# Unalome81/IEEE-802.11-OFDM-QPSK-Simulator

Hardware: NVIDIA B200
Metric: OFDM symbols/s, TX+AWGN+RX chain (BER/EVM sweep) (higher is better)
Workload: dtype f32+f64

## Files before the change

### ieee-802.11-ofdm-qpsk-simulator_b200/csrc/ofdm_sweep.cuh

```cuda
#pragma once
#include "ofdm_chain.cuh"

namespace ofdm {

struct SweepParams {
    const float2 *in;
    const float *g;
    const float *power;
    const uint32_t *tx_bits;
    long n_frames;
    int n_snr;
    float radius_scale;
    float evm_guard;
    float snr_lin[kMaxSnr];
    ofdm_counters *counters;
    unsigned long long *replayed;
};

struct alignas(16) SweepWarp {
    float2 tile[kWarpTile];
    float2 fx[4][kWin];
    float2 fn[4][kWin];
    StreamStage<true> st[kStages];
    uint64_t bar[kStages];
    float norm[8];
};
static_assert(sizeof(SweepWarp) % 16 == 0 && offsetof(SweepWarp, st) % 16 == 0 && offsetof(SweepWarp, norm) % 16 == 0, "SweepWarp alignment");

__device__ __forceinline__ float modulus_up(float2 z)
{
    float r;
    asm("sqrt.approx.ftz.f32 %0, %1;" : "=f"(r) : "f"(fmaf(z.x, z.x, z.y * z.y)));
    return fmaf(r, 1.000004f, 2e-19f);
}

__constant__ unsigned char c_sweep_pair[32] = { 1,  2,  5,  8, 11, 16, 19, 41, 44, 45, 46, 52, 54, 55, 58, 63,
                                                3,  4, 10, 12, 17, 18, 22, 23, 25, 47, 48, 53, 56, 59, 61, 62};
__constant__ unsigned char c_sweep_single[16] = { 6, 14, 15, 20, 26, 40, 49, 50,    9, 13, 24, 38, 39, 42, 51, 60};

struct SweepItems {
    int bin[2];
    int f_off[3];
    float k4[3];
    int word[3];
    int shift[3];
};

__device__ __forceinline__ SweepItems make_sweep_items(int lane)
{
    SweepItems c;
    c.bin[0] = c_sweep_pair[lane];
    c.bin[1] = c_sweep_single[(lane >> 4) * 8 + (lane & 7)];
#pragma unroll
    for (int t = 0; t < 3; ++t) {
        const int bin = c.bin[t >> 1], sym = t == 2 ? (lane >> 3) & 1 : t;
        const int d = c_tab.bin_data[bin];
        c.f_off[t] = sym * kWin + bin;
        c.k4[t] = 4.f * (0.5f * (float)c_tab.bin_lts[bin]);
        c.word[t] = sym * 3 + (d >> 4);
        c.shift[t] = 2 * (d & 15);
    }
    return c;
}

constexpr int kSweepWarps = 6;

template <int ARITH>
__global__ void __launch_bounds__(kSweepWarps * 32, 2) k_sweep_lin(SweepParams p)
{
    constexpr int LEVEL = ARITH == kArithChecked ? 2 : 1;
    constexpr int kWarps = kSweepWarps;
    extern __shared__ __align__(128) unsigned char s_raw[];
    const int lane = threadIdx.x & 31, warp = threadIdx.x >> 5, grp = lane >> 3, u = lane & 7;
    const int warp_u = __shfl_sync(0xffffffffu, warp, 0);
    SweepWarp &ws = reinterpret_cast<SweepWarp *>(s_raw)[warp];
    SweepWarp &ws_u = reinterpret_cast<SweepWarp *>(s_raw)[warp_u];
    float2 *tile = ws.tile + grp * kGroupPitch;
    Tw<false> tw; tw.load(u);
    const SweepItems ic = make_sweep_items(lane);
    constexpr int len = 320;
    const long stride = (long)gridDim.x * kWarps;
    const long f_first = (long)blockIdx.x * kWarps + warp_u;
    const double q = (double)kQpsk;
    const double ref2_frame = 96.0 * (2.0 * q * q);
    const float inv_ref2 = (float)(1.0 / ref2_frame);
    constexpr uint32_t kBytes = 4 * 512 + 4 * 256;
    constexpr int kStep = 3;

    const uint32_t stage0 = tma::saddr(&ws_u.st[0]);
    const uint32_t bar0 = tma::saddr(&ws_u.bar[0]);
    auto issue = [&](long f, int s) {
        if (tma::elect_one()) {
            const uint32_t bar = bar0 + 8u * (uint32_t)s;
            const uint32_t dst = stage0 + (uint32_t)s * (uint32_t)sizeof(StreamStage<true>);
            const char *x = reinterpret_cast<const char *>(p.in) + f * (len * 8);
            const char *g = reinterpret_cast<const char *>(p.g) + f * (len * 4);
            const uint32_t gd = dst + 4 * kWin * 8;
            tma::expect_tx_addr(bar, kBytes);
            tma::bulk_addr(dst + 0 * kWin * 8, x + 32 * 8, 512, bar);
            tma::bulk_addr(dst + 1 * kWin * 8, x + 96 * 8, 512, bar);
            tma::bulk_addr(dst + 2 * kWin * 8, x + 176 * 8, 512, bar);
            tma::bulk_addr(dst + 3 * kWin * 8, x + 256 * 8, 512, bar);
            tma::bulk_addr(gd + 0 * kWin * 4, g + 32 * 4, 256, bar);
            tma::bulk_addr(gd + 1 * kWin * 4, g + 96 * 4, 256, bar);
            tma::bulk_addr(gd + 2 * kWin * 4, g + 176 * 4, 256, bar);
            tma::bulk_addr(gd + 3 * kWin * 4, g + 256 * 4, 256, bar);
        }
    };
    if (lane == 0) {
        for (int s = 0; s < kStages; ++s) tma::mbar_init(&ws.bar[s], 1);
        tma::fence_mbar_init();
    }
    __syncwarp();
    for (int s = 0; s < kStages; ++s)
        if (f_first + s * stride < p.n_frames) issue(f_first + s * stride, s);

    uint32_t m_i[2] = {0, 0}, m_q[2] = {0, 0}, m_b[2] = {0, 0}, m_ferr[2] = {0, 0};
    float m_e2[2] = {0.f, 0.f}, m_evm[2] = {0.f, 0.f};
    double d_e2[2] = {0.0, 0.0}, d_evm[2] = {0.0, 0.0};
    uint32_t n_done = 0;
    uint32_t k = 0;
    for (long f = f_first; f < p.n_frames; f += stride, ++k) {
        const int s = (int)(k & 1u);
        const uint32_t phase = (k >> 1) & 1u;
        const float P = p.power[f];
        const uint32_t *wb = p.tx_bits + f * 6;
        uint32_t txw[3];
#pragma unroll
        for (int t = 0; t < 3; ++t) txw[t] = wb[ic.word[t]];

        tma::wait_addr(bar0 + 8u * (uint32_t)s, phase);
        float2 v[8];
        float gz[8];
        float2 n2x = make_float2(0.f, 0.f);
        float n2g = 0.f;
#pragma unroll
        for (int i = 0; i < 8; ++i) {
            v[i] = ws.st[s].x[grp][u + 8 * i];
            gz[i] = ws.st[s].g[grp][u + 8 * i];
            n2x = __ffma2_rn(v[i], v[i], n2x);
            n2g = fmaf(gz[i], gz[i], n2g);
        }
        __syncwarp();
        if (f + kStages * stride < p.n_frames) issue(f + kStages * stride, s);
        fft64<false>(v, tw, tile, u);
#pragma unroll
        for (int j = 0; j < 8; ++j) ws.fx[grp][u + 8 * j] = v[j];
#pragma unroll
        for (int i = 0; i < 8; ++i) v[i] = make_float2(gz[i], 0.f);
        fft64<false>(v, tw, tile, u);
#pragma unroll
        for (int j = 0; j < 8; ++j) ws.fn[grp][u + 8 * j] = v[j];
        float2 nn = make_float2(n2x.x + n2x.y, n2g);
#pragma unroll
        for (int o = 1; o < 8; o <<= 1)
            nn = __fadd2_rn(nn, make_float2(__shfl_xor_sync(0xffffffffu, nn.x, o), __shfl_xor_sync(0xffffffffu, nn.y, o)));
        {
            float rx, rn;
            asm("sqrt.approx.ftz.f32 %0, %1;" : "=f"(rx) : "f"(nn.x));
            asm("sqrt.approx.ftz.f32 %0, %1;" : "=f"(rn) : "f"(nn.y));
            const bool ok = nn.x >= 1e-30f && nn.x < 1e20f && nn.y < 1e20f;
            const float inf = __int_as_float(0x7f800000);
            if (u == 0) { ws.norm[grp] = ok ? p.radius_scale * rx : inf; ws.norm[4 + grp] = ok ? p.radius_scale * rn : inf; }
        }
        __syncwarp();
        const float4 rX = *reinterpret_cast<const float4 *>(ws.norm), rN = *reinterpret_cast<const float4 *>(ws.norm + 4);
        const float rHX = rX.x + rX.y, rHN = rN.x + rN.y;
        float2 FX[3], FN[3], GX[2], GN[2];
        float c0[3], c1[3], c2[3], hcX[2], hcN[2];
#pragma unroll
        for (int e = 0; e < 2; ++e) {
            const int bin = ic.bin[e];
            GX[e] = cadd(ws.fx[0][bin], ws.fx[1][bin]);
            GN[e] = cadd(ws.fn[0][bin], ws.fn[1][bin]);
            if (LEVEL >= 2) { hcX[e] = modulus_up(GX[e]); hcN[e] = modulus_up(GN[e]); }
        }
#pragma unroll
        for (int t = 0; t < 3; ++t) {
            FX[t] = (&ws.fx[2][0])[ic.f_off[t]];
            FN[t] = (&ws.fn[2][0])[ic.f_off[t]];
            const bool sym0 = ic.f_off[t] < kWin;
            const float rFX = sym0 ? rX.z : rX.w, rFN = sym0 ? rN.z : rN.w;
            if (LEVEL >= 2) {
                const float faX = modulus_up(FX[t]), faN = modulus_up(FN[t]);
                const float hX = hcX[t >> 1], hN = hcN[t >> 1];
                const float A0 = hX + rHX, A1 = hN + rHN;
                c0[t] = fmaf(rFX, A0, fmaf(rHX, faX, 1.2e-7f * (faX * hX)));
                c1[t] = fmaf(rFX, A1, fmaf(rFN, A0, fmaf(rHX, faN, fmaf(rHN, faX, 1.2e-7f * fmaf(faX, hN, faN * hX)))));
                c2[t] = fmaf(rFN, A1, fmaf(rHN, faN, 1.2e-7f * (faN * hN)));
            } else { c0[t] = c1[t] = c2[t] = 0.f; }
        }
        __syncwarp();
        uint32_t gq[3];
#pragma unroll
        for (int t = 0; t < 3; ++t) {
            const uint32_t tp = txw[t] >> ic.shift[t];
            const uint32_t kb = __float_as_uint(ic.k4[t]) & 0x80000000u;
            const uint32_t fq = (tp << 31) ^ kb, fi = ((tp ^ (tp >> 1)) << 31) ^ kb;
            gq[t] = (tp >> 1) << 31;
            FX[t] = make_float2(__uint_as_float(__float_as_uint(FX[t].x) ^ fi), __uint_as_float(__float_as_uint(FX[t].y) ^ fq));
            FN[t] = make_float2(__uint_as_float(__float_as_uint(FN[t].x) ^ fi), __uint_as_float(__float_as_uint(FN[t].y) ^ fq));
        }
#pragma unroll
        for (int e = 0; e < 2; ++e) {
            GX[e].y = __uint_as_float(__float_as_uint(GX[e].y) ^ gq[2 * e]);
            GN[e].y = __uint_as_float(__float_as_uint(GN[e].y) ^ gq[2 * e]);
        }
        const uint32_t g_rel = gq[0] ^ gq[1];
        float sig_lo = 0.f, sig_hi = 0.f;
        if (lane < p.n_snr) sig_lo = __fsqrt_rn(__fdiv_rn(P, p.snr_lin[lane]));
        if (p.n_snr > 32 && lane + 32 < p.n_snr) sig_hi = __fsqrt_rn(__fdiv_rn(P, p.snr_lin[lane + 32]));
        auto sig_pos = [](int i) { return (i / 3) * 4 + i % 3; };
        float *sigs = reinterpret_cast<float *>(&ws.fn[1][0]);
        sigs[sig_pos(lane)] = sig_lo; sigs[sig_pos(lane + 32)] = sig_hi;
        if (lane < 2) sigs[sig_pos(64 + lane)] = 0.f;
        __syncwarp();

        uint2 *res = reinterpret_cast<uint2 *>(&ws.fn[0][0]);
        const float g2_limit = p.radius_scale * 1.58e6f;
        struct PointState { float sg, rH2, den_min4; float2 e2v; uint32_t pk; bool doubt; float2 G; float den, inv; };
        auto point_begin = [&](float sg) {
            PointState q;
            q.sg = sg;
            q.rH2 = fmaf(sg, rHN, rHX);
            const float gd = p.evm_guard * q.rH2;
            q.den_min4 = gd * gd;
            q.e2v = make_float2(0.f, 0.f);
            q.pk = 0; q.doubt = !(q.rH2 < g2_limit);
            return q;
        };
        auto point_item = [&](PointState &q, int t) {
            const float2 sg2 = make_float2(q.sg, q.sg);
            if (t != 1) {
                q.G = __ffma2_rn(sg2, GN[t >> 1], GX[t >> 1]);
                q.den = fmaf(q.G.x, q.G.x, q.G.y * q.G.y);
                asm("rcp.approx.ftz.f32 %0, %1;" : "=f"(q.inv) : "f"(q.den));
            }
            const float2 G = t == 1 ? make_float2(q.G.x, __uint_as_float(__float_as_uint(q.G.y) ^ g_rel)) : q.G;
            const float2 F = __ffma2_rn(sg2, FN[t], FX[t]);
            const float thr = fmaf(fmaf(c2[t], q.sg, c1[t]), q.sg, c0[t]);
            q.pk += process_bin_spec_den<LEVEL, true>(F, G, q.den, q.inv, 2.f, 0u, thr, q.rH2, q.den_min4, q.e2v, q.doubt);
        };
        uint32_t pk_raw[kStep];
        float e2_pend[kStep], red[kStep], red_in[kStep];
#pragma unroll
        for (int j = 0; j < kStep; ++j) { pk_raw[j] = 0; e2_pend[j] = 0.f; }
        auto red_issue = [&](int o) {
#pragma unroll
            for (int j = 0; j < kStep; ++j) red_in[j] = __shfl_xor_sync(0xffffffffu, red[j], o);
        };
        auto red_take = [&]() {
#pragma unroll
            for (int j = 0; j < kStep; ++j) red[j] += red_in[j];
        };
        uint64_t doubt_mask = 0;
        for (int si = 0, sk = 0; si < p.n_snr; si += kStep, sk += 4) {
            uint32_t pk_sum[kStep];
#pragma unroll
            for (int j = 0; j < kStep; ++j) { pk_sum[j] = __reduce_add_sync(0xffffffffu, pk_raw[j]); red[j] = e2_pend[j]; }
            red_issue(16);
            PointState q[kStep];
            const float4 sp = *reinterpret_cast<const float4 *>(sigs + sk);
            q[0] = point_begin(sp.x); q[1] = point_begin(sp.y); q[2] = point_begin(sp.z);
#pragma unroll
            for (int t = 0; t < 3; ++t) {
#pragma unroll
                for (int j = 0; j < kStep; ++j) {
                    const int n = t * kStep + j;
                    point_item(q[j], t);
                    if (n < 4) { red_take(); red_issue(8 >> n); }
                    else if (n == 4) red_take();
                }
            }
            if (lane == 0 && si > 0) {
#pragma unroll
                for (int j = 0; j < kStep; ++j) res[si - kStep + j] = make_uint2(pk_sum[j], __float_as_uint(red[j]));
            }
            uint32_t bits = 0;
#pragma unroll
            for (int j = 0; j < kStep; ++j) {
                pk_raw[j] = q[j].pk;
                e2_pend[j] = q[j].e2v.x + q[j].e2v.y;
                bits |= (uint32_t)q[j].doubt << j;
            }
            doubt_mask |= (uint64_t)bits << si;
        }
        {
            const int last = (p.n_snr - 1) / kStep * kStep;
#pragma unroll
            for (int j = 0; j < kStep; ++j) {
                const uint32_t pk_sum = __reduce_add_sync(0xffffffffu, pk_raw[j]);
                float r = e2_pend[j];
#pragma unroll
                for (int o = 16; o > 0; o >>= 1) r += __shfl_xor_sync(0xffffffffu, r, o);
                if (lane == 0) res[last + j] = make_uint2(pk_sum, __float_as_uint(r));
            }
        }
        {
            if (p.n_snr < 64) doubt_mask &= (1ull << p.n_snr) - 1ull;
            uint64_t todo = __reduce_or_sync(0xffffffffu, (uint32_t)doubt_mask);
            if (p.n_snr > 32) todo |= (uint64_t)__reduce_or_sync(0xffffffffu, (uint32_t)(doubt_mask >> 32)) << 32;
            __syncwarp();
            while (todo != 0) {
                const int si = __ffsll((long long)todo) - 1;
                todo &= todo - 1;
                const float sg = sigs[sig_pos(si)];
                bool replay = true;
                if (LEVEL >= 2) {
                    const float4 qX = *reinterpret_cast<const float4 *>(ws.norm), qN = *reinterpret_cast<const float4 *>(ws.norm + 4);
                    const float2 sg2 = make_float2(sg, sg);
                    const float rH2 = fmaf(sg, rHN, rHX);
                    const float gd = p.evm_guard * rH2, den_min4 = gd * gd;
                    bool doubt2 = false;
                    float2 e2w = make_float2(0.f, 0.f);
                    float2 G;
#pragma unroll
                    for (int t = 0; t < 3; ++t) {
                        if (t != 1) G = __ffma2_rn(sg2, GN[t >> 1], GX[t >> 1]);
                        const float2 Gt = t == 1 ? make_float2(G.x, __uint_as_float(__float_as_uint(G.y) ^ g_rel)) : G;
                        const float2 F = __ffma2_rn(sg2, FN[t], FX[t]);
                        const bool sym0 = ic.f_off[t] < kWin;
                        const float rF = fmaf(sg, sym0 ? qN.z : qN.w, sym0 ? qX.z : qX.w);
                        const float fa = modulus_up(F), hc = modulus_up(Gt);
                        const float thr = fmaf(rF, hc + rH2, fmaf(rH2, fa, 1.2e-7f * (fa * hc)));
                        process_bin_spec<LEVEL, true>(F, Gt, 2.f, 0u, thr, rH2, den_min4, e2w, doubt2);
                    }
                    replay = __any_sync(0xffffffffu, doubt2);
                }
                if (replay) {
                    const double sigma_d = __dsqrt_rn((double)__fdiv_rn(P, p.snr_lin[si]));
                    const uint2 r = stream_frame_replay<kNoiseInject>(p.in + f * len, p.g + f * len, wb, sigma_d, 0u, 0u, 0ull,
                                                                      ws.tile, &ws.fx[0][0], p.replayed);
                    const uint32_t pk_sum = __reduce_add_sync(0xffffffffu, r.x);
                    float e2 = __uint_as_float(r.y);
#pragma unroll
                    for (int o = 16; o > 0; o >>= 1) e2 += __shfl_xor_sync(0xffffffffu, e2, o);
                    if (lane == 0) res[si] = make_uint2(pk_sum, __float_as_uint(e2));
                }
            }
        }
        __syncwarp();
#pragma unroll
        for (int h = 0; h < 2; ++h) {
            if (h == 1 && p.n_snr <= 32) break;
            const uint2 r = res[lane + 32 * h];
            const bool mine = lane + 32 * h < p.n_snr;
            const uint32_t pk = mine ? r.x : 0u;
            const float e2 = mine ? __uint_as_float(r.y) : 0.f;
            float evm;
            asm("sqrt.approx.ftz.f32 %0, %1;" : "=f"(evm) : "f"(e2 * inv_ref2));
            m_i[h] += pk & 0xFFu; m_q[h] += (pk >> 8) & 0xFFu; m_b[h] += pk >> 16; m_ferr[h] += pk != 0u;
            m_e2[h] += e2; m_evm[h] += evm;
        }
        n_done += 1;
        if ((n_done & 63u) == 0u) {
#pragma unroll
            for (int h = 0; h < 2; ++h) { d_e2[h] += (double)m_e2[h]; d_evm[h] += (double)m_evm[h]; m_e2[h] = 0.f; m_evm[h] = 0.f; }
        }
    }
    if (n_done == 0) return;
#pragma unroll
    for (int h = 0; h < 2; ++h) {
        const int si = lane + 32 * h;
        if (si >= p.n_snr) continue;
        ofdm_counters *o = p.counters + si;
        const unsigned long long ti = m_i[h], tq = m_q[h], tb = m_b[h];
        atomicAdd(reinterpret_cast<unsigned long long *>(&o->bit_errors), ti + 2ull * tq - 2ull * tb);
        atomicAdd(reinterpret_cast<unsigned long long *>(&o->rail_errors), ti + tq);
        atomicAdd(reinterpret_cast<unsigned long long *>(&o->frames_in_error), (unsigned long long)m_ferr[h]);
        atomicAdd(reinterpret_cast<unsigned long long *>(&o->frames), (unsigned long long)n_done);
        atomicAdd(reinterpret_cast<unsigned long long *>(&o->bits), 192ull * n_done);
        atomicAdd(&o->sum_err2, d_e2[h] + (double)m_e2[h]);
        atomicAdd(&o->sum_ref2, ref2_frame * (double)n_done);
        atomicAdd(&o->sum_evm_lin, d_evm[h] + (double)m_evm[h]);
    }
}

inline size_t sweep_smem_bytes(int warps) { return sizeof(SweepWarp) * warps; }

}
```

Measured before the change: 10.61 billion.

## Replace per-SNR shuffle reductions with shared-memory transpose and specialized item kernel

Replaces the interleaved butterfly shuffle reduction of EVM partials with per-lane writes of partials into a shared-memory matrix, then each lane sums its own SNR row with paired float adds. Adds a specialized inlined sweep_item that computes the decision, margin and error with packed float2 ops, and folds the doubt check into a three-way NaN-propagating min over margins. Enlarges the per-warp shared struct with dedicated sig and pk arrays, which raises shared memory use and may reduce occupancy. Replay results are now held in the owning lane's registers instead of a shared result array.

```diff
diff --git a/ieee-802.11-ofdm-qpsk-simulator_b200/csrc/ofdm_sweep.cuh b/ieee-802.11-ofdm-qpsk-simulator_b200/csrc/ofdm_sweep.cuh
--- a/ieee-802.11-ofdm-qpsk-simulator_b200/csrc/ofdm_sweep.cuh
+++ b/ieee-802.11-ofdm-qpsk-simulator_b200/csrc/ofdm_sweep.cuh
@@ -17,21 +17,50 @@
     unsigned long long *replayed;
 };
 
+constexpr int kSweepRows = kMaxSnr + 2;
+constexpr int kPartPitch = 36;
+constexpr int kSweepSlots = (kMaxSnr + 2) / 3 * 4;
+
 struct alignas(16) SweepWarp {
     float2 tile[kWarpTile];
     float2 fx[4][kWin];
     float2 fn[4][kWin];
+    float part_tail[kSweepRows * kPartPitch - 2 * (kWarpTile + 8 * kWin)];
+    float sig[kSweepSlots];
+    uint32_t pk[kSweepSlots];
     StreamStage<true> st[kStages];
     uint64_t bar[kStages];
     float norm[8];
 };
-static_assert(sizeof(SweepWarp) % 16 == 0 && offsetof(SweepWarp, st) % 16 == 0 && offsetof(SweepWarp, norm) % 16 == 0, "SweepWarp alignment");
+static_assert(sizeof(SweepWarp) % 16 == 0 && offsetof(SweepWarp, st) % 16 == 0 && offsetof(SweepWarp, norm) % 16 == 0 &&
+              offsetof(SweepWarp, sig) % 16 == 0 && offsetof(SweepWarp, pk) % 16 == 0, "SweepWarp alignment");
+static_assert(offsetof(SweepWarp, part_tail) == 2 * (kWarpTile + 8 * kWin) * sizeof(float) &&
+              offsetof(SweepWarp, sig) == kSweepRows * kPartPitch * sizeof(float), "the partials run from tile to sig");
 
 __device__ __forceinline__ float modulus_up(float2 z)
 {
     float r;
     asm("sqrt.approx.ftz.f32 %0, %1;" : "=f"(r) : "f"(fmaf(z.x, z.x, z.y * z.y)));
     return fmaf(r, 1.000004f, 2e-19f);
+}
+
+__device__ __forceinline__ uint32_t sweep_item(float2 F, float2 G, float inv, float thr, float &margin, float2 &e2)
+{
+    const float2 pt = __fmul2_rn(make_float2(G.y, G.y), make_float2(F.y, F.x));
+    const float2 S = __ffma2_rn(make_float2(G.x, G.x), F, make_float2(pt.x, -pt.y));
+    const uint32_t ei = __float_as_uint(S.x) >> 31, eq = __float_as_uint(S.y) >> 31;
+    margin = fminf(fabsf(S.x), fabsf(S.y)) - thr;
+    const float2 U = __fmul2_rn(S, make_float2(inv, inv));
+    const float2 D = __ffma2_rn(U, make_float2(2.f, 2.f), make_float2(__uint_as_float(0xBF3504F3u), __uint_as_float(0xBF3504F3u)));
+    e2 = __ffma2_rn(D, D, e2);
+    return ei | (eq << 8) | ((ei & eq) << 16);
+}
+
+__device__ __forceinline__ float min3_nan(float a, float b, float c)
+{
+    float r;
+    asm("min.NaN.f32 %0, %1, %2, %3;" : "=f"(r) : "f"(a), "f"(b), "f"(c));
+    return r;
 }
 
 __constant__ unsigned char c_sweep_pair[32] = { 1,  2,  5,  8, 11, 16, 19, 41, 44, 45, 46, 52, 54, 55, 58, 63,
@@ -211,14 +240,14 @@
         if (lane < p.n_snr) sig_lo = __fsqrt_rn(__fdiv_rn(P, p.snr_lin[lane]));
         if (p.n_snr > 32 && lane + 32 < p.n_snr) sig_hi = __fsqrt_rn(__fdiv_rn(P, p.snr_lin[lane + 32]));
         auto sig_pos = [](int i) { return (i / 3) * 4 + i % 3; };
-        float *sigs = reinterpret_cast<float *>(&ws.fn[1][0]);
+        float *sigs = ws.sig;
         sigs[sig_pos(lane)] = sig_lo; sigs[sig_pos(lane + 32)] = sig_hi;
         if (lane < 2) sigs[sig_pos(64 + lane)] = 0.f;
         __syncwarp();
 
-        uint2 *res = reinterpret_cast<uint2 *>(&ws.fn[0][0]);
+        float *const part = reinterpret_cast<float *>(ws.tile);
         const float g2_limit = p.radius_scale * 1.58e6f;
-        struct PointState { float sg, rH2, den_min4; float2 e2v; uint32_t pk; bool doubt; float2 G; float den, inv; };
+        struct PointState { float sg, rH2, den_min4; float2 e2v; uint32_t pk; bool doubt; float2 G; float den, inv, m0, m1; };
         auto point_begin = [&](float sg) {
             PointState q;
             q.sg = sg;
@@ -235,72 +264,75 @@
                 q.G = __ffma2_rn(sg2, GN[t >> 1], GX[t >> 1]);
                 q.den = fmaf(q.G.x, q.G.x, q.G.y * q.G.y);
                 asm("rcp.approx.ftz.f32 %0, %1;" : "=f"(q.inv) : "f"(q.den));
+                q.doubt = q.doubt || !(q.den > q.den_min4);
             }
             const float2 G = t == 1 ? make_float2(q.G.x, __uint_as_float(__float_as_uint(q.G.y) ^ g_rel)) : q.G;
             const float2 F = __ffma2_rn(sg2, FN[t], FX[t]);
-            const float thr = fmaf(fmaf(c2[t], q.sg, c1[t]), q.sg, c0[t]);
-            q.pk += process_bin_spec_den<LEVEL, true>(F, G, q.den, q.inv, 2.f, 0u, thr, q.rH2, q.den_min4, q.e2v, q.doubt);
+            const float thr = LEVEL >= 2 ? fmaf(fmaf(c2[t], q.sg, c1[t]), q.sg, c0[t]) : 0.f;
+            float m;
+            q.pk += sweep_item(F, G, q.inv, thr, m, q.e2v);
+            if (LEVEL >= 2) {
+                if (t == 0) q.m0 = m;
+                else if (t == 1) q.m1 = m;
+                else q.doubt = q.doubt || !(min3_nan(q.m0, q.m1, m) > 2e-30f);
+            }
         };
         uint32_t pk_raw[kStep];
-        float e2_pend[kStep], red[kStep], red_in[kStep];
-#pragma unroll
-        for (int j = 0; j < kStep; ++j) { pk_raw[j] = 0; e2_pend[j] = 0.f; }
-        auto red_issue = [&](int o) {
-#pragma unroll
-            for (int j = 0; j < kStep; ++j) red_in[j] = __shfl_xor_sync(0xffffffffu, red[j], o);
-        };
-        auto red_take = [&]() {
-#pragma unroll
-            for (int j = 0; j < kStep; ++j) red[j] += red_in[j];
-        };
+#pragma unroll
+        for (int j = 0; j < kStep; ++j) pk_raw[j] = 0;
         uint64_t doubt_mask = 0;
         for (int si = 0, sk = 0; si < p.n_snr; si += kStep, sk += 4) {
             uint32_t pk_sum[kStep];
 #pragma unroll
-            for (int j = 0; j < kStep; ++j) { pk_sum[j] = __reduce_add_sync(0xffffffffu, pk_raw[j]); red[j] = e2_pend[j]; }
-            red_issue(16);
+            for (int j = 0; j < kStep; ++j) pk_sum[j] = __reduce_add_sync(0xffffffffu, pk_raw[j]);
             PointState q[kStep];
             const float4 sp = *reinterpret_cast<const float4 *>(sigs + sk);
             q[0] = point_begin(sp.x); q[1] = point_begin(sp.y); q[2] = point_begin(sp.z);
 #pragma unroll
             for (int t = 0; t < 3; ++t) {
 #pragma unroll
-                for (int j = 0; j < kStep; ++j) {
-                    const int n = t * kStep + j;
-                    point_item(q[j], t);
-                    if (n < 4) { red_take(); red_issue(8 >> n); }
-                    else if (n == 4) red_take();
-                }
-            }
-            if (lane == 0 && si > 0) {
-#pragma unroll
-                for (int j = 0; j < kStep; ++j) res[si - kStep + j] = make_uint2(pk_sum[j], __float_as_uint(red[j]));
-            }
+                for (int j = 0; j < kStep; ++j) point_item(q[j], t);
+            }
+            if (lane == 0 && si > 0) *reinterpret_cast<uint4 *>(ws.pk + sk - 4) = make_uint4(pk_sum[0], pk_sum[1], pk_sum[2], 0u);
             uint32_t bits = 0;
 #pragma unroll
             for (int j = 0; j < kStep; ++j) {
+                part[(si + j) * kPartPitch + lane] = q[j].e2v.x + q[j].e2v.y;
                 pk_raw[j] = q[j].pk;
-                e2_pend[j] = q[j].e2v.x + q[j].e2v.y;
                 bits |= (uint32_t)q[j].doubt << j;
             }
             doubt_mask |= (uint64_t)bits << si;
         }
         {
-            const int last = (p.n_snr - 1) / kStep * kStep;
-#pragma unroll
-            for (int j = 0; j < kStep; ++j) {
-                const uint32_t pk_sum = __reduce_add_sync(0xffffffffu, pk_raw[j]);
-                float r = e2_pend[j];
-#pragma unroll
-                for (int o = 16; o > 0; o >>= 1) r += __shfl_xor_sync(0xffffffffu, r, o);
-                if (lane == 0) res[last + j] = make_uint2(pk_sum, __float_as_uint(r));
-            }
-        }
+            const int last = (p.n_snr - 1) / kStep * 4;
+            uint32_t pk_sum[kStep];
+#pragma unroll
+            for (int j = 0; j < kStep; ++j) pk_sum[j] = __reduce_add_sync(0xffffffffu, pk_raw[j]);
+            if (lane == 0) *reinterpret_cast<uint4 *>(ws.pk + last) = make_uint4(pk_sum[0], pk_sum[1], pk_sum[2], 0u);
+        }
+        __syncwarp();
+        uint32_t pk_own[2];
+        float e2_own[2];
+#pragma unroll
+        for (int h = 0; h < 2; ++h) {
+            pk_own[h] = 0u; e2_own[h] = 0.f;
+            if (h == 1 && p.n_snr <= 32) break;
+            const float4 *row = reinterpret_cast<const float4 *>(part + (lane + 32 * h) * kPartPitch);
+            float2 a = make_float2(0.f, 0.f), b = make_float2(0.f, 0.f);
+#pragma unroll
+            for (int c = 0; c < 8; ++c) {
+                const float4 v = row[c];
+                a = __fadd2_rn(a, make_float2(v.x, v.y));
+                b = __fadd2_rn(b, make_float2(v.z, v.w));
+            }
+            e2_own[h] = (a.x + a.y) + (b.x + b.y);
+            pk_own[h] = ws.pk[sig_pos(lane + 32 * h)];
+        }
+        __syncwarp();
         {
             if (p.n_snr < 64) doubt_mask &= (1ull << p.n_snr) - 1ull;
             uint64_t todo = __reduce_or_sync(0xffffffffu, (uint32_t)doubt_mask);
             if (p.n_snr > 32) todo |= (uint64_t)__reduce_or_sync(0xffffffffu, (uint32_t)(doubt_mask >> 32)) << 32;
-            __syncwarp();
             while (todo != 0) {
                 const int si = __ffsll((long long)todo) - 1;
                 todo &= todo - 1;
@@ -335,18 +367,19 @@
                     float e2 = __uint_as_float(r.y);
 #pragma unroll
                     for (int o = 16; o > 0; o >>= 1) e2 += __shfl_xor_sync(0xffffffffu, e2, o);
-                    if (lane == 0) res[si] = make_uint2(pk_sum, __float_as_uint(e2));
+                    if (lane == (si & 31)) {
+                        if (si < 32) { pk_own[0] = pk_sum; e2_own[0] = e2; }
+                        else         { pk_own[1] = pk_sum; e2_own[1] = e2; }
+                    }
                 }
             }
         }
-        __syncwarp();
 #pragma unroll
         for (int h = 0; h < 2; ++h) {
             if (h == 1 && p.n_snr <= 32) break;
-            const uint2 r = res[lane + 32 * h];
             const bool mine = lane + 32 * h < p.n_snr;
-            const uint32_t pk = mine ? r.x : 0u;
-            const float e2 = mine ? __uint_as_float(r.y) : 0.f;
+            const uint32_t pk = mine ? pk_own[h] : 0u;
+            const float e2 = mine ? e2_own[h] : 0.f;
             float evm;
             asm("sqrt.approx.ftz.f32 %0, %1;" : "=f"(evm) : "f"(e2 * inv_ref2));
             m_i[h] += pk & 0xFFu; m_q[h] += (pk >> 8) & 0xFFu; m_b[h] += pk >> 16; m_ferr[h] += pk != 0u;
```

Result: faster. 11.24 billion, median of 6 (+6.0%).
